# DerekRowell/AudioSDR

Hardware: AMD Instinct MI355X
Metric: Msamples/s through full SSB demod chain, batched 128-sample blocks (higher is better)
Workload: dtype f32

## Files before the change

audiosdr_amd/csrc/asdr_fir.h:

```cpp
#ifndef ASDR_FIR_H
#define ASDR_FIR_H
#include <hip/hip_runtime.h>

typedef float v2f __attribute__((ext_vector_type(2)));
#ifndef ASDR_FIR_TAPS_IN_VGPRS
#define ASDR_FIR_TAPS_IN_VGPRS 0
#endif
#ifndef SCHED_FENCE
#define SCHED_FENCE() do { } while (0)
#endif

template <int E0, int NE, bool TAPS_V = (ASDR_FIR_TAPS_IN_VGPRS != 0)>
__device__ __forceinline__ void hilbert_fir_rows(const float *hist, int p0, v2f *acc2, const float *taps) {
  constexpr int NW = NE + 7;
  const v2f *PX = reinterpret_cast<const v2f *>(hist) + E0;
#pragma unroll 1
  for (int kc = 0; kc < 8; ++kc) {
    v2f dw[NW], uw[NW];
    const float4 *dp = reinterpret_cast<const float4 *>(PX + 120 + p0 - 8 * kc);
    const float4 *up = reinterpret_cast<const float4 *>(PX + p0 + 8 * kc);
#pragma unroll
    for (int q = 0; q < NW / 2; ++q) {
      const float4 d4 = dp[q], u4 = up[q];
      dw[2 * q] = (v2f){d4.x, d4.y}; dw[2 * q + 1] = (v2f){d4.z, d4.w};
      uw[2 * q] = (v2f){u4.x, u4.y}; uw[2 * q + 1] = (v2f){u4.z, u4.w};
    }
    if (NW & 1) { dw[NW - 1] = PX[120 + p0 - 8 * kc + NW - 1]; uw[NW - 1] = PX[p0 + 8 * kc + NW - 1]; }
#pragma unroll
    for (int kk = 0; kk < 8; ++kk) {
      float hk = taps[8 * kc + kk];
      if constexpr (TAPS_V) asm("" : "+v"(hk));
      const v2f hk2 = (v2f){hk, hk};
      v2f d[NE];
#pragma unroll
      for (int e = 0; e < NE; ++e) d[e] = dw[7 + e - kk] - uw[e + kk];
#pragma unroll
      for (int e = 0; e < NE; ++e) d[e] = hk2 * d[e];
#pragma unroll
      for (int e = 0; e < NE; ++e) acc2[e] += d[e];
      SCHED_FENCE();
    }
  }
}
#endif
```

audiosdr_amd/csrc/asdr_kernels.hip:

```cpp
#include <hip/hip_runtime.h>
#include <stdint.h>
#include <stddef.h>
#include <string.h>
#include <stdlib.h>
#include <type_traits>

#include "asdr_device.h"
#include "asdr_tables.h"
#include "../../include/asdr.h"

#define W0 0
#define W1 128
#define PH 256
#define XP 0
#ifndef ASDR_STRIDE
#define ASDR_STRIDE 388
#endif
#ifndef ASDR_AGC_QUIET_PATH
#define ASDR_AGC_QUIET_PATH 1
#endif
#ifndef ASDR_MW_OWN_STORES
#define ASDR_MW_OWN_STORES 1
#endif
#ifndef ASDR_AGC_LEAN
// ... 481 lines not shown
}
__device__ __forceinline__ float als_group_sum_tail(float y, const AlsGroup &G, int rem) {
  float p0 = G.w.x * G.x0, p1 = G.w.y * G.x1, p2 = G.w.z * G.x2, p3 = G.w.w * G.x3;
  p0 = (0 < rem) ? p0 : 0.0f; p1 = (2 < rem) ? p1 : 0.0f; p2 = (4 < rem) ? p2 : 0.0f; p3 = (6 < rem) ? p3 : 0.0f;
  y += p0; y += dpp_row_shl4(p0); y += p1; y += dpp_row_shl4(p1);
  y += p2; y += dpp_row_shl4(p2); y += p3; y += dpp_row_shl4(p3);
  return y;
}
__device__ __forceinline__ float als_dot_split(const float *wh, const float *xh, int M, int h) {
  float y = 0.0f;
  const int n_full = M >> 3;
  AlsGroup A;
  for (int g = 0; g < n_full; ++g) { als_group_load(A, wh, xh, g); y = als_group_sum(y, A); }
  if (M & 7) { als_group_load(A, wh, xh, n_full); y = als_group_sum_tail(y, A, (M & 7) - h); }
  return y;
}
__device__ __forceinline__ float als_dot_split_uniform(const float *wh, const float *xh, int M, int h) {
  float y = 0.0f;
  const int n_full = M >> 3, rem = (M & 7) - h;
  AlsGroup A, B;
  als_group_load(A, wh, xh, 0);
  int g = 0;
#pragma unroll 1
  for (; g + 2 <= n_full; g += 2) {
    als_group_load(B, wh, xh, g + 1);
    __builtin_amdgcn_sched_barrier(0);
    y = als_group_sum(y, A);
    als_group_load(A, wh, xh, g + 2);
    __builtin_amdgcn_sched_barrier(0);
    y = als_group_sum(y, B);
  }
  if (g < n_full) {
    als_group_load(B, wh, xh, g + 1);
    __builtin_amdgcn_sched_barrier(0);
    y = als_group_sum(y, A);
    if (M & 7) y = als_group_sum_tail(y, B, rem);
  } else if (M & 7) {
    y = als_group_sum_tail(y, A, rem);
  }
  return y;
}

#define ALS_M_DEFAULT 55
template <int MC>
__device__ __forceinline__ float als_dot_split_const(const float *wh, const float *xh, int h) {
  constexpr int NF = MC >> 3, R = MC & 7, NG = NF + (R ? 1 : 0);
  float y = 0.0f;
  AlsGroup G[2];
  als_group_load(G[0], wh, xh, 0);
#pragma unroll
  for (int g = 0; g < NF; ++g) {
    if (g + 1 < NG) als_group_load(G[(g + 1) & 1], wh, xh, g + 1);
    __builtin_amdgcn_sched_barrier(0);
    y = als_group_sum(y, G[g & 1]);
  }
  if (R) y = als_group_sum_tail(y, G[NF & 1], R - h);
  return y;
}
template <int MC>
__device__ __forceinline__ void als_tap_update_const(const float *xq, float *wq, float e, float lam, int s8) {
  constexpr int NF = MC >> 3, R = MC & 7, NK = NF + (R ? 1 : 0);
  float xv[NK], wv[NK];
#pragma unroll
  for (int k = 0; k < NK; ++k) { xv[k] = xq[-8 * k]; wv[k] = wq[4 * k]; }
#pragma unroll
  for (int k = 0; k < NK; ++k) {
    const float gq = e * xv[k]; const float dq = lam * gq; const float wn = wv[k] + dq;
    wv[k] = (k < NF || s8 < R) ? wn : wv[k];
  }
#pragma unroll
  for (int k = 0; k < NK; ++k) wq[4 * k] = wv[k];
}

#define DEFINE_ALL_PATHS(arr, n) do { _Pragma("unroll") for (int z_ = 0; z_ < (n); ++z_) (arr)[z_] = 0.0f; } while (0)
template <typename T>
__device__ __forceinline__ T *row_ptr(T *base, uint32_t byte_off) {
  return reinterpret_cast<T *>(reinterpret_cast<char *>(base) + byte_off);
}
template <typename T>
__device__ __forceinline__ const T *row_ptr(const T *base, uint32_t byte_off) {
  return reinterpret_cast<const T *>(reinterpret_cast<const char *>(base) + byte_off);
}
#define WAVE_SYNC() do { __builtin_amdgcn_fence(__ATOMIC_RELEASE, "workgroup"); __builtin_amdgcn_wave_barrier(); \
                         __builtin_amdgcn_fence(__ATOMIC_ACQUIRE, "workgroup"); } while (0)

#ifndef ASDR_PLL_CONSTS_IN_VGPRS
#define ASDR_PLL_CONSTS_IN_VGPRS 1
#endif
template <bool TWO_SUMS, int CH, bool PF = false, typename LD, typename ST>
__device__ __forceinline__ bool pll_loop(ChanSmall *Sc, const ChainConsts &K_, const float *sine, float two_pi, LD ld, ST st) {
    ChainConsts K = K_;
    if constexpr (PF && ASDR_PLL_CONSTS_IN_VGPRS) {
      asm("" : "+v"(K.pll_a1), "+v"(K.pll_b0), "+v"(K.pll_b1), "+v"(K.half_pi_f), "+v"(two_pi), "+v"(K.pll_alpha_freq), "+v"(K.pll_beta_freq), "+v"(K.pll_f_conv),
               "+v"(K.pll_lock_lo), "+v"(K.pll_lock_hi));
      asm("" : "+v"(K.sin_index_scale_d), "+v"(K.half_pi_d));
    }
    float y_re = Sc->pll_y_re, y_im = Sc->pll_y_im, prev_filt = Sc->pll_prev_filt;
    float d0 = Sc->pll_d0, d1 = Sc->pll_d1, phase_est = Sc->pll_phase_est, pfreq = Sc->pll_freq;
    bool locked = false;
    float nr[CH], ni[CH];
    if (PF) ld(0, nr, ni);
#pragma unroll 1
    for (int i = 0; i < ASDR_N; i += CH) {
      float xr[CH], xi[CH];
      if (PF) {
#pragma unroll
        for (int u = 0; u < CH; ++u) { xr[u] = nr[u]; xi[u] = ni[u]; }
        ld((i + CH < ASDR_N) ? i + CH : i, nr, ni);
      } else {
        ld(i, xr, xi);
      }
#pragma unroll
      for (int u = 0; u < CH; ++u) {
        const float x_re = xr[u], x_im = xi[u];
        const float d_re = x_re * y_re + x_im * y_im;
        const float d_im = x_im * y_re - x_re * y_im;
        const float err = approx_atan2<TWO_SUMS>(d_im, d_re, K.half_pi_f);
        d1 = d0;
        d0 = err - K.pll_a1 * d1;
        const float filt = K.pll_b0 * d0 + K.pll_b1 * d1;
        phase_est = __builtin_fmaf(filt + prev_filt, 0.5f, phase_est);
        prev_filt = filt;
        { const float pi_up = 3.14159274101257324f;
          const float turned = phase_est - __builtin_copysignf(two_pi, phase_est);
          phase_est = (fabsf(phase_est) >= pi_up) ? turned : phase_est;
          if (__any(fabsf(phase_est) >= pi_up)) {
            int turns = 1;
            while (phase_est >= pi_up && turns < ASDR_PLL_WRAP_MAX) { phase_est -= two_pi; ++turns; }
            while (phase_est <= -pi_up && turns < ASDR_PLL_WRAP_MAX) { phase_est += two_pi; ++turns; }
            if (turns >= ASDR_PLL_WRAP_MAX) phase_est = 0.0f;
          } }
#ifndef ASDR_PLL_FLAT_LOOKUPS
        sincos_pll(sine, phase_est, y_re, y_im, two_pi, SinIndexK{K.inv_two_pi_d, K.sin_index_scale_d}, K.half_pi_d);
#else
        y_re = cos_f32<true>(sine, phase_est, two_pi, SinIndexK{K.inv_two_pi_d, K.sin_index_scale_d}, K.half_pi_d);
        y_im = sin_f32<true>(sine, phase_est, two_pi, SinIndexK{K.inv_two_pi_d, K.sin_index_scale_d});
#endif
        pfreq = K.pll_alpha_freq * pfreq + K.pll_beta_freq * (filt * K.pll_f_conv);
        locked = (pfreq > K.pll_lock_lo) && (pfreq < K.pll_lock_hi);
        const float o_re = x_re * y_re + x_im * y_im, o_im = -x_re * y_im + x_im * y_re;
        xr[u] = locked ? o_re : x_re;
        xi[u] = locked ? o_im : x_im;
      }
      st(i, xr, xi);
    }
    Sc->pll_y_re = y_re; Sc->pll_y_im = y_im; Sc->pll_prev_filt = prev_filt;
    Sc->pll_d0 = d0; Sc->pll_d1 = d1; Sc->pll_phase_est = phase_est; Sc->pll_freq = pfreq;
    return locked;
}

template <int E0, int NE, bool TAPS_V = (ASDR_FIR_TAPS_IN_VGPRS != 0)>
__device__ __forceinline__ void hilbert_fir(const float *Lrow, int p0, v2f *acc2) {
  hilbert_fir_rows<E0, NE, TAPS_V>(Lrow + XP, p0, acc2, c_hilbert);
}
template <int STRIDE, int E0 = 4, int NE = 4>
__device__ __forceinline__ void asdr_stream_fir_helper(const UpdateArgs &a, float *lds) {
  const int lane = threadIdx.x & 63, c8 = lane >> 3, s8 = lane & 7, k0 = 16 * s8;
  float *L = lds + c8 * STRIDE;
  const int wave_g = (int)blockIdx.x % a.stream_waves;
  if (((a.direct_ch0 >= 0) ? a.direct_mode : a.sched[wave_g * 8].mode) == ASDR_AMmode) return;
#pragma unroll 1
  for (int blk = 0; blk < a.n_blocks; ++blk) {
    v2f acc2[NE];
#pragma unroll
    for (int e = 0; e < NE; ++e) acc2[e] = (v2f){0.0f, 0.0f};
    __syncthreads();
    if (ABL_ON(ABL_HIL)) hilbert_fir<E0, NE>(L, k0 >> 1, acc2);
    __syncthreads();
#pragma unroll
    for (int e = 0; e < NE; e += 2) *reinterpret_cast<float4 *>(L + W1 + k0 + 2 * (E0 + e)) = make_float4(acc2[e][0], acc2[e][1], acc2[e + 1][0], acc2[e + 1][1]);
    __syncthreads();
  }
}

__device__ __forceinline__ uint32_t stream_wait(const uint32_t *p, uint32_t target, uint32_t *err, uint32_t limit) {
  uint32_t spins = 0, v;
  while ((v = __hip_atomic_load(p, __ATOMIC_RELAXED, __HIP_MEMORY_SCOPE_AGENT)) < target) {
    __builtin_amdgcn_s_sleep(2);
    ++spins;
    if (spins > limit) { __hip_atomic_store(err, 1u, __ATOMIC_RELAXED, __HIP_MEMORY_SCOPE_AGENT); v = ASDR_STREAM_FAIL; break; }
    if ((spins & 63u) == 0u && __hip_atomic_load(err, __ATOMIC_RELAXED, __HIP_MEMORY_SCOPE_AGENT) != 0u) { v = ASDR_STREAM_FAIL; break; }
  }
  asm volatile("" ::: "memory");
  return v;
}
__device__ __forceinline__ void stream_signal(uint32_t *p, uint32_t value, int lane) {
  asm volatile("s_waitcnt vmcnt(0)" ::: "memory");
  if (lane == 0) __hip_atomic_store(p, value, __ATOMIC_RELAXED, __HIP_MEMORY_SCOPE_AGENT);
}
__device__ __forceinline__ v4f ld_sc1_v4(const float *p) {
  const unsigned long long lo = __hip_atomic_load(reinterpret_cast<const unsigned long long *>(p), __ATOMIC_RELAXED, __HIP_MEMORY_SCOPE_AGENT);
  const unsigned long long hi = __hip_atomic_load(reinterpret_cast<const unsigned long long *>(p) + 1, __ATOMIC_RELAXED, __HIP_MEMORY_SCOPE_AGENT);
  v4f r;
  r[0] = __uint_as_float((uint32_t)lo); r[1] = __uint_as_float((uint32_t)(lo >> 32)); r[2] = __uint_as_float((uint32_t)hi); r[3] = __uint_as_float((uint32_t)(hi >> 32));
  return r;
}
__device__ __forceinline__ void xch_store4x4(float *p, v4f v0, v4f v1, v4f v2, v4f v3) {
  asm volatile("global_store_dwordx4 %0, %1, off sc1\n\tglobal_store_dwordx4 %0, %2, off offset:128 sc1\n\t"
               "global_store_dwordx4 %0, %3, off offset:256 sc1\n\tglobal_store_dwordx4 %0, %4, off offset:384 sc1\n\t"
               "s_nop 1"
               :: "v"(p), "v"(v0), "v"(v1), "v"(v2), "v"(v3) : "memory");
}
__device__ __forceinline__ void xch_load4x4(const float *p, v4f &v0, v4f &v1, v4f &v2, v4f &v3) {
  asm volatile("global_load_dwordx4 %0, %4, off sc1\n\tglobal_load_dwordx4 %1, %4, off offset:128 sc1\n\t"
               "global_load_dwordx4 %2, %4, off offset:256 sc1\n\tglobal_load_dwordx4 %3, %4, off offset:384 sc1\n\t"
               "s_waitcnt vmcnt(0)"
               : "=&v"(v0), "=&v"(v1), "=&v"(v2), "=&v"(v3) : "v"(p) : "memory");
}

template <bool COMPACT, int XB, int AW, int WH, int SCR, int OUT>
__device__ __forceinline__ void als_compute(float *L, bool als_en, bool adaptive, bool notch, int M, int D, float lam, int s8, int k0) {
    constexpr int AH = 2 * WH;
    const bool als_safe = COMPACT || __all(!als_en || (D >= 0 && D + M <= AH + 1));
    const int M_u = __builtin_amdgcn_readfirstlane(M);
    const bool als_m_uniform = __all(als_en && adaptive && M == M_u);
    const bool als_m_default = als_m_uniform && als_safe && M_u == ALS_M_DEFAULT;
    if (__any(als_en && !adaptive)) {
      float yo[16];
#pragma unroll
      for (int j = 0; j < 16; ++j) yo[j] = 0.0f;
      if (als_en && !adaptive) {
        for (int j = 0; j < 16; ++j) {
          const int i = 128 + k0 + j;
          float y;
          if constexpr (COMPACT) y = als_dot<false, WH>(L + AW, L + XB, i - D, M);
          else y = als_safe ? als_dot<false, WH>(L + AW, L + XB, i - D, M) : als_dot<true, WH>(L + AW, L + XB, i - D, M);
          const float e = L[XB + i] - y;
          yo[j] = notch ? e : y;
        }
      }
      WAVE_SYNC();
      if (als_en && !adaptive) {
#pragma unroll
        for (int j = 0; j < 16; ++j) L[OUT + k0 + j] = yo[j];
      }
    }
#ifndef ASDR_ALS_TAPS_IN_LDS
    if (als_m_default) {
      const int h = s8 >> 2, tq = s8 & 3;
      float wr[7];
#pragma unroll
      for (int g = 0; g < 7; ++g) wr[g] = L[AW + WH * h + 4 * g + tq];
      const bool own_valid6 = !(tq == 3 && h != 0);
      auto epoch = [&](auto first_tag, auto j_tag, int ep, const float *E, const float *F, const float *XI) {
        constexpr bool FIRST = decltype(first_tag)::value;
        constexpr int J = decltype(j_tag)::value;
        const int base = FIRST ? 0 : 4 * ep + 1;
        const int cntn = FIRST ? 1 : ((ep == 31) ? 3 : 4);
        const int n = base + tq, i = 128 + n;
        const bool mine = (s8 < cntn);
        const int nu = FIRST ? 0 : 4 * ep + 4;
        float xs[7][4], xo[7], xi;
        if constexpr (J < 0) {
          const float *xh = L + XB + (i - D - h);
#pragma unroll
          for (int g = 0; g < 7; ++g) { xs[g][0] = xh[-8 * g]; xs[g][1] = xh[-8 * g - 2]; xs[g][2] = xh[-8 * g - 4]; xs[g][3] = xh[-8 * g - 6]; }
          const float *xu = L + XB + (128 + nu - D - h - 2 * tq);
#pragma unroll
          for (int g = 0; g < 7; ++g) xo[g] = xu[-8 * g];
          xi = L[XB + i];
        } else {
#pragma unroll
          for (int g = 0; g < 7; ++g) {
#pragma unroll
            for (int t = 0; t < 4; ++t) xs[g][t] = E[6 + 4 * g + t - 2 * J];
            xo[g] = F[3 + 2 * g - J];
          }
          xi = XI[J];
        }
        float y = 0.0f;
#pragma unroll
        for (int g = 0; g < 7; ++g) {
          float p[4];
          p[0] = __int_as_float(__builtin_amdgcn_update_dpp(0, __float_as_int(wr[g]), 0x00, 0xF, 0xF, true)) * xs[g][0];
          p[1] = __int_as_float(__builtin_amdgcn_update_dpp(0, __float_as_int(wr[g]), 0x55, 0xF, 0xF, true)) * xs[g][1];
          p[2] = __int_as_float(__builtin_amdgcn_update_dpp(0, __float_as_int(wr[g]), 0xAA, 0xF, 0xF, true)) * xs[g][2];
          p[3] = __int_as_float(__builtin_amdgcn_update_dpp(0, __float_as_int(wr[g]), 0xFF, 0xF, 0xF, true)) * xs[g][3];
          if (g == 6) p[3] = (h == 0) ? p[3] : 0.0f;
#pragma unroll
          for (int t = 0; t < 4; ++t) { y += p[t]; y += dpp_row_shl4(p[t]); }
#ifdef ASDR_ALS_GROUP_BARRIER
          __builtin_amdgcn_sched_barrier(0);
#endif
        }
#ifndef ASDR_ALS_SUMS_SINKABLE
        asm volatile("" : "+v"(y));
#endif
        float e_own = 0.0f;
        if (mine) {
          e_own = xi - y;
          L[OUT + n] = notch ? e_own : y;
        }
        if (nu < ASDR_N) {
          const int eq = __builtin_amdgcn_update_dpp(0, __float_as_int(e_own), FIRST ? 0x00 : 0xFF, 0xF, 0xF, true);
          const float e = __int_as_float(__builtin_amdgcn_update_dpp(eq, eq, 0x114, 0xF, 0xA, false));
#pragma unroll
          for (int g = 0; g < 7; ++g) {
            const float gq = e * xo[g]; const float dq = lam * gq; const float wn = wr[g] + dq;
            wr[g] = (g == 6 && !own_valid6) ? wr[g] : wn;
          }
        }
      };
      epoch(std::true_type{}, std::integral_constant<int, -1>{}, -1, nullptr, nullptr, nullptr);
#if ASDR_ALS_WINDOW
#pragma unroll 1
      for (int grp = 0; grp < 8; ++grp) {
// ... 1100 lines not shown
              mq[j] = vq[j] * cc[j] + vi[j] * sn[j];                                                                                          \
            }                                                                                                                                 \
            if (qn_direct) {                                                                                                                  \
              _Pragma("unroll")                                                                                                               \
              for (int j = 0; j < 4; ++j) qn[4 * m + j] = mq[j];                                                                              \
            } else { store4(L + W0 + kF + 32 * m, mi); store4(L + W1 + kF + 32 * m, mq); }                                                    \
            store4_nt(hi_ring + hs * 128 + 32 * m, mi);                                                                                       \
          }
        if (lo_hit || mix_uni) { C16_MIX_LOOP(true) }
        else {
          DEFINE_ALL_PATHS(hq_o, 16); DEFINE_ALL_PATHS(hq_m, 16);
          C16_MIX_LOOP(false)
#pragma unroll
          for (int m = 0; m < 4; ++m) { load4(hq_ring + hs * 128 + 32 * m, hq_o + 4 * m); load4(hq_ring + (hs ^ 1u) * 128 + 32 * m, hq_m + 4 * m); }
        }
      }
    } else
    if (ABL_ON(ABL_MIX) && do_mix) {
#pragma unroll
      for (int m = 0; m < 4; ++m) {
        float cc[4], sn[4], vi[4], vq[4], mi[4], mq[4];
        load4(L + W0 + kF + 32 * m, vi); load4(L + W1 + kF + 32 * m, vq);
        if (lo_hit) {
          if (RING_PREFETCH) {
#pragma unroll
            for (int j = 0; j < 4; ++j) { cc[j] = lo_c[4 * m + j]; sn[j] = lo_s[4 * m + j]; }
          } else { load4(lo_rd->c + kF + 32 * m, cc); load4(lo_rd->s + kF + 32 * m, sn); }
        } else if (mix_uni) {
          load4(lds + STRIDE + PH + kF + 32 * m, cc); load4(lds + 2 * STRIDE + PH + kF + 32 * m, sn);
        } else {
          float ph[4];
          load4(L + PH + kF + 32 * m, ph);
#ifndef ASDR_MIX_SERIAL_LOOKUPS
          sincos_batch<4, SINE_LDS_PC>(SINE_LDS_PC ? sine_tab : nullptr, ph, cc, sn, two_pi, SinIndexK{K.inv_two_pi_d, K.sin_index_scale_d}, K.half_pi_d);
#else
#pragma unroll
          for (int j = 0; j < 4; ++j) {
            cc[j] = cos_f32(sine, ph[j], two_pi, SinIndexK{K.inv_two_pi_d, K.sin_index_scale_d}, K.half_pi_d); sn[j] = sin_f32(sine, ph[j], two_pi, SinIndexK{K.inv_two_pi_d, K.sin_index_scale_d});
            if ((j & 1) == 1) SCHED_FENCE();
          }
#endif
        }
#pragma unroll
        for (int j = 0; j < 4; ++j) {
          mi[j] = vi[j] * cc[j] - vq[j] * sn[j];
          mq[j] = vq[j] * cc[j] + vi[j] * sn[j];
        }
        if (qn_direct) {
#pragma unroll
          for (int j = 0; j < 4; ++j) qn[4 * m + j] = mq[j];
        } else { store4(L + W0 + kF + 32 * m, mi); store4(L + W1 + kF + 32 * m, mq); }
#ifndef ASDR_TEMPORAL_RINGS
        if (is_ssb) store4_nt(hi_ring + hs * 128 + 32 * m, mi);
#else
        if (is_ssb) store4(hi_ring + hs * 128 + 32 * m, mi);
#endif
      }
    }

    float4 af_s4 = make_float4(0.f, 0.f, 0.f, 0.f);
    float af_cf[5] = {0.f, 0.f, 0.f, 0.f, 0.f};
    float agc_gain_in = 0.f, agc_old0 = 0.f, agc_carrier0 = 0.f;
    uint32_t agc_hc0 = 0u;
    int agc_tab_idx = 0;
    const bool mw_audio_duty = (MW_SHARE & 1) && (mw_rel == 1 || mw_rel == 2);
    const int mw_casc = PLB ? (4 * (lane_i >> 4) + (lane_i & 3)) : (lane_i >> 2);
    ChanSmall *mw_af_S = S;
    auto load_af_agc_state = [&]() {
    ChanSmall *const Saf = PLB ? Spa : S; const ChanParams *const Paf = PLB ? Ppa : Pp;
    if (ABL_ON(ABL_AF) && (((MW_SHARE & 1) != 0) ? af_en : af_en_pa)) {
      if constexpr ((MW_SHARE & 1) != 0) {
        if (mw_audio_duty) {
          const int chq = mw_channel(16 * (mw_rel - 1) + mw_casc);
          mw_af_S = row_ptr(a.small, (uint32_t)chq * (uint32_t)sizeof(ChanSmall));
          af_s4 = *reinterpret_cast<const float4 *>(&mw_af_S->af_state[4 * pl_st]);
          const float *cf = &c_bq_pool[(UPAR ? &a.uni : row_ptr(a.params, (uint32_t)chq * (uint32_t)sizeof(ChanParams)))->audio_table][5 * pl_st];
#pragma unroll
          for (int z = 0; z < 5; ++z) af_cf[z] = cf[z];
        }
      } else {
      af_s4 = *reinterpret_cast<const float4 *>(&Saf->af_state[4 * pl_st]);
      const float *cf = &c_bq_pool[Paf->audio_table][5 * pl_st];
#pragma unroll
      for (int z = 0; z < 5; ++z) af_cf[z] = cf[z];
      }
    }
    if (ABL_ON(ABL_AGC) && agc_en) {
      agc_gain_in = S->agc_gain; agc_old0 = S->agc_old_abs; agc_hc0 = S->agc_hang_counter; agc_carrier0 = S->am_carrier;
      agc_tab_idx = P.agc_table;
    }
    };
    if constexpr (!C16) load_af_agc_state();
    TL(7);
    if (__any(is_ssb)) {
      if (is_ssb && !qn_direct) {
#pragma unroll
        for (int m = 0; m < 4; ++m) load4(L + W1 + kF + 32 * m, qn + 4 * m);
      }
      WAVE_SYNC();
      if constexpr (C16) {
#pragma unroll
        for (int m = 0; m < 4; ++m) {
#pragma unroll
          for (int j = 0; j < 4; ++j) {
            const int k = kF + 32 * m + j;
            if (k >= 1) L[XP + k - 1] = hq_o[4 * m + j];
            L[XP + 127 + k] = hq_m[4 * m + j];
            if (k < 63) L[XP + 255 + k] = qn[4 * m + j];
          }
          store4_nt(hq_ring + hs * 128 + 32 * m, qn + 4 * m);
        }
        if (lead) S->hil_slot = hs ^ 1u;
        WAVE_SYNC();
        TL(8);
        v2f fa[4], fb[4];
#pragma unroll
        for (int e = 0; e < 4; ++e) { fa[e] = (v2f){0.0f, 0.0f}; fb[e] = (v2f){0.0f, 0.0f}; }
        if (ABL_ON(ABL_HIL)) hilbert_fir<0, 4, false>(L, 4 * s8, fa);
        WAVE_SYNC();
        {
          float t[32];
#pragma unroll
          for (int q = 0; q < 8; ++q) load4(L + XP + 64 + 32 * s8 + 4 * q, t + 4 * q);
          WAVE_SYNC();
#pragma unroll
          for (int q = 0; q < 8; ++q) store4(L + XP + 32 * s8 + 4 * q, t + 4 * q);
        }
#pragma unroll
        for (int m = 0; m < 4; ++m) {
#pragma unroll
          for (int j = 0; j < 4; ++j) { const int k = kF + 32 * m + j; if (k >= 63 && k < 127) L[XP + 191 + k] = qn[4 * m + j]; }
        }
        WAVE_SYNC();
        if (ABL_ON(ABL_HIL)) hilbert_fir<0, 4, false>(L, 4 * s8, fb);
        WAVE_SYNC();
        TL(9);
        load_af_agc_state();
#pragma unroll
        for (int m = 0; m < 4; ++m) load4(hi_ring + (hs ^ 1u) * 128 + 32 * m, idl + 4 * m);
        *reinterpret_cast<float4 *>(L + W1 + 8 * s8) = make_float4(fa[0][0], fa[0][1], fa[1][0], fa[1][1]);
        *reinterpret_cast<float4 *>(L + W1 + 8 * s8 + 4) = make_float4(fa[2][0], fa[2][1], fa[3][0], fa[3][1]);
        *reinterpret_cast<float4 *>(L + W1 + 64 + 8 * s8) = make_float4(fb[0][0], fb[0][1], fb[1][0], fb[1][1]);
        *reinterpret_cast<float4 *>(L + W1 + 64 + 8 * s8 + 4) = make_float4(fb[2][0], fb[2][1], fb[3][0], fb[3][1]);
        WAVE_SYNC();
      } else {
      if (is_ssb) {
        if (!RING_PREFETCH) {
#pragma unroll
          for (int m = 0; m < 4; ++m) {
            load4(hq_ring + hs * 128 + 32 * m, hq_o + 4 * m);
            load4(hq_ring + (hs ^ 1u) * 128 + 32 * m, hq_m + 4 * m);
          }
        }
#pragma unroll
        for (int m = 0; m < 4; ++m) {
#pragma unroll
          for (int j = 0; j < 4; ++j) {
            const int k = kF + 32 * m + j;
            if (k >= 1) L[XP + k - 1] = hq_o[4 * m + j];
            L[XP + 127 + k] = hq_m[4 * m + j];
          }
        }
#pragma unroll
        for (int m = 0; m < 4; ++m) {
#pragma unroll
          for (int j = 0; j < 4; ++j) L[XP + 255 + kF + 32 * m + j] = qn[4 * m + j];
#ifndef ASDR_TEMPORAL_RINGS
          store4_nt(hq_ring + hs * 128 + 32 * m, qn + 4 * m);
#else
          store4(hq_ring + hs * 128 + 32 * m, qn + 4 * m);
#endif
        }
        if (lead) S->hil_slot = hs ^ 1u;
        carry_hs = hs ^ 1u;
      }
      WAVE_SYNC();
      TL(8);
      mw_straggler(3);
      if constexpr (R2_PREFETCH) {
        const uint32_t b2 = (uint32_t)blk + 2u;
        if (blk + 1 < a.n_blocks && (seen_in < b2 || seen_lo < b2)) {
          const uint32_t ui = (uint32_t)__builtin_amdgcn_readfirstlane((int)r2_look_in), ul = (uint32_t)__builtin_amdgcn_readfirstlane((int)r2_look_lo);
          asm volatile("" ::: "memory");
          if (ui != ASDR_STREAM_FAIL && ui > seen_in) seen_in = ui;
          if (ul != ASDR_STREAM_FAIL && ul > seen_lo) seen_lo = ul;
        }
        if (blk + 1 < a.n_blocks && seen_in != ASDR_STREAM_FAIL && seen_lo != ASDR_STREAM_FAIL && seen_in >= b2 && seen_lo >= b2) {
          const LoEntry *ln = a.lo_ring + ((blk + 1) % ASDR_LO_RING);
          const float *lp = ln->c + kF, *xp = a.xch_a + ((size_t)ch * ASDR_STREAM_DEPTH + (size_t)((blk + 1) % ASDR_STREAM_DEPTH)) * (2 * ASDR_N) + kF;
          r2n_key = ld_sc1_v4(reinterpret_cast<const float *>(ln));
#pragma unroll
          for (int m = 0; m < 4; ++m) { r2n_c4[m] = ld_sc1_v4(lp + 32 * m); r2n_s4[m] = ld_sc1_v4(lp + ASDR_N + 32 * m); r2n_vi[m] = ld_sc1_v4(xp + 32 * m); r2n_vq[m] = ld_sc1_v4(xp + ASDR_N + 32 * m); }
          r2_pref = true;
        }
      }
#ifndef ASDR_UPAR_IDL_EARLY
#define ASDR_UPAR_IDL_EARLY 1
#endif
      constexpr bool IDL_EARLY = (ROLE == 2) || (UPAR && ASDR_UPAR_IDL_EARLY != 0);
      if (IDL_EARLY && is_ssb) {
#pragma unroll
        for (int m = 0; m < 4; ++m) load4(hi_ring + (hs ^ 1u) * 128 + 32 * m, idl + 4 * m);
      }
      constexpr int FIR_NE = (ROLE == 2) ? 8 / (FIR_HELPERS + 1) : 8;
      v2f acc2[FIR_NE];
#pragma unroll
      for (int e = 0; e < FIR_NE; ++e) acc2[e] = (v2f){0.0f, 0.0f};
      if (ROLE == 2) __syncthreads();
      if (ABL_ON(ABL_HIL) && is_ssb) hilbert_fir<0, FIR_NE>(L, k0 >> 1, acc2);
      if (ROLE == 2) __syncthreads(); else WAVE_SYNC();
      TL(9);
      if (!IDL_EARLY && is_ssb) {
#pragma unroll
        for (int m = 0; m < 4; ++m) {
#if ASDR_NT_LOADS >= 4
          load4_nt(hi_ring + (hs ^ 1u) * 128 + 32 * m, idl + 4 * m);
#else
          load4(hi_ring + (hs ^ 1u) * 128 + 32 * m, idl + 4 * m);
#endif
        }
      }
      if (is_ssb) {
#pragma unroll
        for (int e = 0; e < FIR_NE; e += 2) *reinterpret_cast<float4 *>(L + W1 + k0 + 2 * e) = make_float4(acc2[e][0], acc2[e][1], acc2[e + 1][0], acc2[e + 1][1]);
      }
      if (ROLE == 2) __syncthreads(); else WAVE_SYNC();
      }
      if (is_ssb) {
        const uint32_t sgn = sub_q ? 0x80000000u : 0u;
#pragma unroll
        for (int m = 0; m < 4; ++m) {
          float qh[4], au[4];
          load4(L + W1 + kF + 32 * m, qh);
#pragma unroll
          for (int j = 0; j < 4; ++j) au[j] = idl[4 * m + j] + __uint_as_float(__float_as_uint(qh[j]) ^ sgn);
          store4(L + W0 + kF + 32 * m, au);
          TAP4(ASDR_TAP_MIX_I, m, idl + 4 * m); TAP4(ASDR_TAP_MIX_Q, m, qh);
        }
      }
    }

    if (ABL_ON(ABL_ENV) && __any(do_env)) {
      WAVE_SYNC();
      {
        const int iq = pl_iq, st = pl_st;
        const bool do_env_p = PLB ? (__builtin_amdgcn_ds_bpermute(pl_c << 5, do_env ? 1 : 0) != 0) : do_env;
        float sv[4];
        ChanSmall *const Simg = Sp;
        const float4 s4 = *reinterpret_cast<const float4 *>(&Simg->img_state[iq][4 * st]);
        sv[0] = s4.x; sv[1] = s4.y; sv[2] = s4.z; sv[3] = s4.w;
        biquad_pipe<PIPE_PK>(Lp + (iq ? W1 : W0), do_env_p, st, &c_bq_pool[ASDR_TBL_AM_IMAGE][5 * st], sv);
        if (do_env_p) *reinterpret_cast<float4 *>(&Simg->img_state[iq][4 * st]) = make_float4(sv[0], sv[1], sv[2], sv[3]);
      }
      WAVE_SYNC();
      if (do_env) {
#pragma unroll 1
        for (int h = 0; h < 2; ++h) {
          float vi[8], vq[8], au[8];
          load8(L + W0 + kA + 64 * h, vi); load8(L + W1 + kA + 64 * h, vq);
          TAP8(ASDR_TAP_MIX_I, h, vi); TAP8(ASDR_TAP_MIX_Q, h, vq);
#pragma unroll
          for (int j = 0; j < 8; ++j) { au[j] = sqrtf(vi[j] * vi[j] + vq[j] * vq[j]); if ((j & 3) == 3) SCHED_FENCE(); }
          store8(L + W0 + kA + 64 * h, au);
        }
      }
      WAVE_SYNC();
      if (do_env && lead) {
        float lvl = S->am_carrier;
#pragma unroll 1
        for (int i = 0; i < ASDR_N; i += 4) {
          const float4 x4 = *reinterpret_cast<const float4 *>(L + W0 + i);
          lvl = (float)(.995 * (double)lvl + 0.005 * (double)fabsf(x4.x));
          lvl = (float)(.995 * (double)lvl + 0.005 * (double)fabsf(x4.y));
          lvl = (float)(.995 * (double)lvl + 0.005 * (double)fabsf(x4.z));
          lvl = (float)(.995 * (double)lvl + 0.005 * (double)fabsf(x4.w));
        }
        S->am_carrier = lvl; carrier_now = lvl; carrier_fresh = true;
        if (ROLE == 2) {
          float *xc = a.xch_c + (size_t)ch * ASDR_STREAM_DEPTH + (size_t)(blk % ASDR_STREAM_DEPTH);
          asm volatile("global_store_dword %0, %1, off sc1\n\ts_nop 0" :: "v"(xc), "v"(lvl) : "memory");
        }
      }
    }
    if (is_sam && pll_locked) {
#pragma unroll 1
      for (int h = 0; h < 2; ++h) {
        float vi[8], vq[8];
        load8(L + W0 + kA + 64 * h, vi); load8(L + W1 + kA + 64 * h, vq);
        TAP8(ASDR_TAP_MIX_I, h, vi); TAP8(ASDR_TAP_MIX_Q, h, vq);
        store8(L + W0 + kA + 64 * h, vq);
      }
    }
    if ((ROLE == 0 || ROLE == 6 || ROLE == 7) && !is_ssb && !is_am && mode != ASDR_SAMmode) {
      float z[16];
      DEFINE_ALL_PATHS(z, 16);
      if (a.audio_prev != nullptr) {
        const float *ap = row_ptr(a.audio_prev, (uint32_t)ch * 512u + 4u * (uint32_t)kF);
#pragma unroll
        for (int m = 0; m < 4; ++m) load4(ap + 32 * m, z + 4 * m);
      }
#pragma unroll
      for (int m = 0; m < 4; ++m) store4(L + W0 + kF + 32 * m, z + 4 * m);
    }
    WAVE_SYNC();
    TL(10);
    TAP_ROW(ASDR_TAP_DEMOD, W0);
    if (ROLE == 2 || ROLE == 3) {
      float *xb = a.xch_b + ((size_t)ch * ASDR_STREAM_DEPTH + (size_t)(blk % ASDR_STREAM_DEPTH)) * ASDR_N + kF;
      if (ROLE == 2) {
        v4f v[4];
#pragma unroll
        for (int m = 0; m < 4; ++m) v[m] = *reinterpret_cast<const v4f *>(L + W0 + kF + 32 * m);
        xch_store4x4(xb, v[0], v[1], v[2], v[3]);
        sig_pending = (uint32_t)blk + 1u;
        continue;
      } else {
        v4f v[4];
        if (is_am) {
          const float *xc = a.xch_c + (size_t)ch * ASDR_STREAM_DEPTH + (size_t)(blk % ASDR_STREAM_DEPTH);
          asm volatile("global_load_dword %4, %6, off sc1\n\t"
                       "global_load_dwordx4 %0, %5, off sc1\n\tglobal_load_dwordx4 %1, %5, off offset:128 sc1\n\t"
                       "global_load_dwordx4 %2, %5, off offset:256 sc1\n\tglobal_load_dwordx4 %3, %5, off offset:384 sc1\n\t"
                       "s_waitcnt vmcnt(0)"
                       : "=&v"(v[0]), "=&v"(v[1]), "=&v"(v[2]), "=&v"(v[3]), "=&v"(carrier_now) : "v"(xb), "v"(xc) : "memory");
          carrier_fresh = true;
        } else
        xch_load4x4(xb, v[0], v[1], v[2], v[3]);
        if (sig_pending) { if (lane == 0) __hip_atomic_store(my_prog, sig_pending, __ATOMIC_RELAXED, __HIP_MEMORY_SCOPE_AGENT); sig_pending = 0u; }
#pragma unroll
        for (int m = 0; m < 4; ++m) *reinterpret_cast<v4f *>(L + W0 + kF + 32 * m) = v[m];
        WAVE_SYNC();
      }
    }

    float4 agc_t4[5];
#pragma unroll
    for (int r = 0; r < 5; ++r) agc_t4[r] = make_float4(0.f, 0.f, 0.f, 0.f);
    float agc_al_a = 0.f, agc_be_a = 0.f, agc_al_r = 0.f, agc_be_r = 0.f, agc_sg = 0.f;
    uint32_t agc_hang = 0u;
    if (ABL_ON(ABL_AGC) && agc_en) {
      agc_al_a = P.agc_alpha_att; agc_be_a = P.agc_beta_att; agc_al_r = P.agc_alpha_rel; agc_be_r = P.agc_beta_rel;
      agc_sg = P.agc_static_gain; agc_hang = P.agc_hang_count;
      const float *gtab = a.agc_tab + (size_t)agc_tab_idx * ASDR_AGC_TAB_ROW;
      if constexpr (!C16) {
#pragma unroll
      for (int r = 0; r < 5; ++r) { const int q = s8 + 8 * r; if (q < 33) agc_t4[r] = reinterpret_cast<const float4 *>(gtab)[q]; }
      }
    }
    if constexpr ((MW_SHARE & 1) != 0) {
      if (ABL_ON(ABL_AF) && af_en) {
        if constexpr (PIPE_AGC) {
          if (agc_piped && lead && agc_en) {
            float *mq = mwx + MWX * (wave * 8 + c8);
            mq[8] = agc_old0; mq[11] = agc_al_a; mq[12] = agc_be_a;
          }
        }
        TL(21);
        if constexpr (MW && (ASDR_MW_STRAGGLER_PRIO != 0 || ASDR_MW_PRIO_REL0_TAIL != 0)) __builtin_amdgcn_s_setprio(0);
        __syncthreads();
        TL(22);
        if (mw_audio_duty) {
#ifndef ASDR_MW_PRIO_AUDIO
// ... 1161 lines not shown
```

Baseline: 85360.

## Use register ring-buffer Hilbert FIR to reuse LDS window loads across taps

Adds a Hilbert FIR variant that keeps a 16-entry rolling register window of down and up history samples. Each pair of taps loads only one new float4 per side, instead of reloading a full window per 8-tap chunk, which cuts LDS read traffic and instruction count. It is enabled by default for the multi-wave 4-wave configuration. A DPP-based vectorized history store path is also added but disabled by default. The register window raises VGPR pressure, and the sched_barrier placement constrains the scheduler.

```diff
diff --git a/audiosdr_amd/csrc/asdr_fir.h b/audiosdr_amd/csrc/asdr_fir.h
--- a/audiosdr_amd/csrc/asdr_fir.h
+++ b/audiosdr_amd/csrc/asdr_fir.h
@@ -42,4 +42,39 @@
     }
   }
 }
+
+__device__ __forceinline__ void hilbert_fir_rows_ring(const float *hist, int p0, v2f *acc2, const float *taps) {
+  constexpr int NE = 8;
+  const v2f *PD = reinterpret_cast<const v2f *>(hist) + 64 + p0;
+  const v2f *PU = reinterpret_cast<const v2f *>(hist) + p0;
+  v2f D[16], U[16];
+  auto ld2 = [](const v2f *p, v2f &a, v2f &b) { const float4 q = *reinterpret_cast<const float4 *>(p); a = (v2f){q.x, q.y}; b = (v2f){q.z, q.w}; };
+#pragma unroll
+  for (int t = 60; t < 72; t += 2) ld2(PD + t, D[t & 15], D[(t + 1) & 15]);
+#pragma unroll
+  for (int t = 0; t < 12; t += 2) ld2(PU + t, U[t], U[t + 1]);
+#pragma unroll 1
+  for (int tc = 0; tc < 4; ++tc) {
+    float h[16];
+#pragma unroll
+    for (int i = 0; i < 16; ++i) h[i] = taps[16 * tc + i];
+#pragma unroll
+    for (int tt = 0; tt < 16; ++tt) {
+      if ((tt & 1) == 0) {
+        ld2(PD + 58 - tt, D[(58 - tt) & 15], D[(59 - tt) & 15]);
+        ld2(PU + 12 + tt, U[(12 + tt) & 15], U[(13 + tt) & 15]);
+      }
+      const v2f hk2 = (v2f){h[tt], h[tt]};
+      v2f d[NE];
+#pragma unroll
+      for (int e = 0; e < NE; ++e) d[e] = D[(63 - tt + e) & 15] - U[(tt + e) & 15];
+#pragma unroll
+      for (int e = 0; e < NE; ++e) d[e] = hk2 * d[e];
+#pragma unroll
+      for (int e = 0; e < NE; ++e) acc2[e] += d[e];
+      if ((tt & 1) == 1) __builtin_amdgcn_sched_barrier(0);
+    }
+    PD -= 16; PU += 16;
+  }
+}
 #endif
diff --git a/audiosdr_amd/csrc/asdr_kernels.hip b/audiosdr_amd/csrc/asdr_kernels.hip
--- a/audiosdr_amd/csrc/asdr_kernels.hip
+++ b/audiosdr_amd/csrc/asdr_kernels.hip
@@ -657,6 +657,29 @@
 template <int E0, int NE, bool TAPS_V = (ASDR_FIR_TAPS_IN_VGPRS != 0)>
 __device__ __forceinline__ void hilbert_fir(const float *Lrow, int p0, v2f *acc2) {
   hilbert_fir_rows<E0, NE, TAPS_V>(Lrow + XP, p0, acc2, c_hilbert);
+}
+#ifndef ASDR_MW_FIR_RING
+#define ASDR_MW_FIR_RING 1
+#endif
+#ifndef ASDR_MW_HIST_B128
+#define ASDR_MW_HIST_B128 0
+#endif
+__device__ __forceinline__ void hilbert_fir_ring(const float *Lrow, int p0, v2f *acc2) {
+  hilbert_fir_rows_ring(Lrow + XP, p0, acc2, c_hilbert);
+}
+template <bool LAST>
+__device__ __forceinline__ void hilbert_hist_store16(float *dst, const float *v, float next0, bool seam) {
+#pragma unroll
+  for (int m = 0; m < 4; ++m) {
+    float w = __int_as_float(__builtin_amdgcn_update_dpp(0, __float_as_int(v[4 * m]), 0x101, 0xF, 0xF, true));
+    float p1 = v[4 * m + 1], p2 = v[4 * m + 2], p3 = v[4 * m + 3];
+    asm volatile("" : "+v"(p1), "+v"(p2), "+v"(p3));
+    if (!(LAST && m == 3)) {
+      const float s = __int_as_float(__builtin_amdgcn_update_dpp(0, __float_as_int(m < 3 ? v[4 * m + 4] : next0), 0x117, 0xF, 0xF, true));
+      w = seam ? s : w;
+    }
+    *reinterpret_cast<float4 *>(dst + 32 * m) = make_float4(p1, p2, p3, w);
+  }
 }
 template <int STRIDE, int E0 = 4, int NE = 4>
 __device__ __forceinline__ void asdr_stream_fir_helper(const UpdateArgs &a, float *lds) {
@@ -2063,6 +2086,14 @@
             load4(hq_ring + (hs ^ 1u) * 128 + 32 * m, hq_m + 4 * m);
           }
         }
+        constexpr bool HIST_B128 = MW && WAVES == 4 && (ASDR_MW_HIST_B128 != 0);
+        if constexpr (HIST_B128) {
+          hilbert_hist_store16<false>(L + XP + kF, hq_o, hq_m[0], s8 == 7);
+          __builtin_amdgcn_sched_barrier(0);
+          hilbert_hist_store16<false>(L + XP + 128 + kF, hq_m, qn[0], s8 == 7);
+          __builtin_amdgcn_sched_barrier(0);
+          hilbert_hist_store16<true>(L + XP + 256 + kF, qn, 0.0f, s8 == 7);
+        } else {
 #pragma unroll
         for (int m = 0; m < 4; ++m) {
 #pragma unroll
@@ -2072,10 +2103,13 @@
             L[XP + 127 + k] = hq_m[4 * m + j];
           }
         }
+        }
 #pragma unroll
         for (int m = 0; m < 4; ++m) {
+          if constexpr (!HIST_B128) {
 #pragma unroll
           for (int j = 0; j < 4; ++j) L[XP + 255 + kF + 32 * m + j] = qn[4 * m + j];
+          }
 #ifndef ASDR_TEMPORAL_RINGS
           store4_nt(hq_ring + hs * 128 + 32 * m, qn + 4 * m);
 #else
@@ -2118,7 +2152,8 @@
 #pragma unroll
       for (int e = 0; e < FIR_NE; ++e) acc2[e] = (v2f){0.0f, 0.0f};
       if (ROLE == 2) __syncthreads();
-      if (ABL_ON(ABL_HIL) && is_ssb) hilbert_fir<0, FIR_NE>(L, k0 >> 1, acc2);
+      if constexpr (MW && WAVES == 4 && ASDR_MW_FIR_RING != 0 && ASDR_FIR_TAPS_IN_VGPRS == 0) { if (ABL_ON(ABL_HIL) && is_ssb) hilbert_fir_ring(L, k0 >> 1, acc2); }
+      else if (ABL_ON(ABL_HIL) && is_ssb) hilbert_fir<0, FIR_NE>(L, k0 >> 1, acc2);
       if (ROLE == 2) __syncthreads(); else WAVE_SYNC();
       TL(9);
       if (!IDL_EARLY && is_ssb) {
```

Result: faster. 86990, median of 6 (+1.9%).
